# plume-sig/zk-nullifier-sig

Hardware: AMD Instinct MI355X
Metric: PLUME verifies/sec (secp256k1 V1) at batch=2^20 per GPU (higher is better)
Workload: dtype u32; 1 GPU; BASELINE.json configs[1]/metric: batch 2^20 per GPU, PLUME V1 verify (secp256k1 + SHA-256), 32-byte messages, 1/16 corrupted, inputs resident in HBM; Fp arithmetic on 9x29-bit limbs through chains of v_mad_u64_u32 (32x32+64); items_per_gpu=1048576, parallelism=shard x1, no collective on the data path, world_size=1

## Files before the change

__graft_entry__.py:

```python
import os
import subprocess
import sys
from pathlib import Path

ROOT = Path(__file__).resolve().parent
os.environ.setdefault("HSA_ENABLE_IPC_MODE_LEGACY", "0")
os.environ.setdefault("GPU_MAX_HW_QUEUES", "8")
if str(ROOT) not in sys.path:
    sys.path.insert(0, str(ROOT))


def build() -> None:
    env = dict(os.environ, PYTORCH_ROCM_ARCH="gfx950")
    subprocess.check_call(["make", "-j2", "-C", str(ROOT / "zk-nullifier-sig_amd" / "csrc")], env=env)
    subprocess.check_call(["make", "-C", str(ROOT / "oracle")])
    subprocess.check_call(["make", "-C", str(ROOT / "tests" / "devsim")])
    subprocess.check_call(["make", "-C", str(ROOT / "tests" / "devgpu")])
    import zk_nullifier_sig_amd as plume
    assert plume.library_path().exists()


def smoke() -> None:
    import numpy as np

    import zk_nullifier_sig_amd as plume
    from oracle import plume_oracle as O
    from tests import _oracle_c as OC
    from tests import synth

    eng = plume.Engine(0)
    n = 64
    for ver in (1, 2):
        b = synth.sign_inputs(n)
        got = eng.sign_batch(ver, b["msgs"], b["off"], b["sk"], b["r"])
        want = OC.sign_batch(ver, b["msgs"], b["off"], b["sk"], b["r"], nthreads=4)
        for k in got:
            assert np.array_equal(got[k], want[k]), f"sign v{ver}: {k} differs from the oracle"
        v = synth.corrupt_for_verify(ver, b, got)
        ok = eng.verify_batch(ver, v["msgs"], v["off"], v["pk"], v["nullifier"], v["c"], v["s"], v.get("r_point"), v.get("hashed_to_curve_r"))
        want_ok = OC.verify_batch(ver, v["msgs"], v["off"], v["pk"], v["nullifier"], v["c"], v["s"], v.get("r_point"), v.get("hashed_to_curve_r"), nthreads=4)
        assert np.array_equal(ok, want_ok), f"verify v{ver} differs from the oracle"
        assert list(ok) == [0 if i % 16 == 5 else 1 for i in range(n)]
        nz = (ver, b["msgs"], b["off"], got["pk"], got["nullifier"], got["s"], got["r_point"], got["hashed_to_curve_r"], got["c"])
        assert np.array_equal(eng.verify_non_zk_batch(*nz), OC.verify_non_zk_batch(*nz, nthreads=4)), f"verify_non_zk v{ver} differs from the oracle"

    class Mock:
        def fill_bytes(self, k):
            return bytes.fromhex("93b9323b629f251b8f3fc2dd11f4672c5544e8230d493eceea98a90bda789808")

    sk = plume.SecretKey.from_bytes(bytes.fromhex("519b423d715f8b581f4fa8ee59f4771a5b44c8130b4e3eacca54a56dda72b464"))
    sig = plume.PlumeSignature.sign_v1(sk, b"An example app message string", Mock(), eng)
    assert sig.c.to_bytes().hex() == "c6a7fc2c926ddbaf20731a479fb6566f2daa5514baae5223fe3b32edbce83254"
    assert sig.s.to_bytes().hex() == "e69f027d84cb6fe5f761e333d12e975fb190d163e8ea132d7de0bd6079ba28ca"
    assert sig.verify(eng)
    assert O.verify(1, sig.message, (sig.pk.x, sig.pk.y), (sig.nullifier.x, sig.nullifier.y), sig.c.value, sig.s.value,
                    (sig.v1specific.r_point.x, sig.v1specific.r_point.y), (sig.v1specific.hashed_to_curve_r.x, sig.v1specific.hashed_to_curve_r.y))
    eng.close()
    print("smoke ok:", plume.library_path())


if __name__ == "__main__":
    build() if (len(sys.argv) < 2 or sys.argv[1] == "build") else smoke()
```

zk-nullifier-sig_amd/csrc/plume_capi.hip:

```cpp
#include <hip/hip_runtime.h>

#include <sched.h>

#include <cctype>
#include <condition_variable>
#include <cstdio>
#include <cstdlib>
#include <cstring>
#include <functional>
#include <iterator>
#include <map>
#include <mutex>
#include <cerrno>
#include <sys/random.h>
#include <string>
#include <thread>
#include <tuple>
#include <initializer_list>
#include <algorithm>
#include <atomic>
#include <memory>
#include <vector>

#include "../../include/plume_hip.h"
// ... 672 lines not shown
}

struct RecoverCall {
    RecoverLaunch fn;
    int version, format;
    uint8_t *rpt, *hr, *h, *status;
};

static int verify_device(plume_ctx* ctx, int version, int mode, size_t n, const uint8_t* msgs, const uint64_t* msg_off, size_t msgs_bytes, const uint8_t* pk, const uint8_t* nul,
                         const uint8_t* c, const uint8_t* s, const uint8_t* rpt, const uint8_t* hr, uint8_t* ok, hipStream_t st,
                         const uint8_t* preflags = nullptr, bool continue_timer = false, const uint8_t* rpt33 = nullptr, const uint8_t* hr33 = nullptr,
                         const RecoverCall* rec = nullptr) {
    if (n == 0) return 0;
    if (n > ctx->chunk) return fail(PLUME_ERR_ARG, "n exceeds the chunk size (plume_set_chunk)");
    if (int rc = need_gtab(ctx)) return rc;
    const bool eq1short = verify_eq1_short(ctx, version, mode, n, rpt != nullptr && rpt33 == nullptr);
    if (eq1short) { if (int rc = need_gcomb(ctx)) return rc; }
    const size_t J = eq1short ? 4 : 3;
    if (!continue_timer) { if (int rc = ws_acquire(ctx, st)) return rc; }
    std::unique_ptr<WsHold> hold(continue_timer ? nullptr : new WsHold(ctx, st));
    const std::vector<size_t> cut = sub_batch_bounds(ctx, n);
    const size_t nsub = cut.size() - 1;
    const bool overlapped = nsub > 1;
    if (int rc = verify_workspace(ctx, n, J, cut)) return rc;
    if (overlapped) { if (int rc = pre_events(ctx, nsub)) return rc; if (int rc = pre_stream(ctx)) return rc; }
    StageTimer& t = ctx->timer;
    if (!continue_timer) t.begin(st);
    hipStream_t pre = overlapped ? ctx->pre : st;
    if (overlapped) {
        HIPCHK(hipEventRecord(ctx->pre_begin, st));
        HIPCHK(hipStreamWaitEvent(pre, ctx->pre_begin, 0));
    }
    for (size_t k = 0; k < nsub; k++) {
        const size_t lo = cut[k], cnt = cut[k + 1] - cut[k];
        VerifyArgs a;
        memset(&a, 0, sizeof a);
        a.version = version; a.mode = mode; a.n = (uint32_t)cnt; a.msgs = msgs; a.msg_off = msg_off + lo; a.msgs_bytes = msgs_bytes;
        a.pk = pk + 64 * lo; a.nul = nul + 64 * lo; a.c = c + 32 * lo; a.s = s + 32 * lo; a.rpt = rpt ? rpt + 64 * lo : nullptr; a.hr = hr ? hr + 64 * lo : nullptr; a.ok = ok ? ok + lo : nullptr;
        a.preflags = preflags ? preflags + lo : nullptr; a.rpt33 = rpt33 ? rpt33 + 33 * lo : nullptr; a.hr33 = hr33 ? hr33 + 33 * lo : nullptr;
        a.bases = ctx->bases.as<uint32_t>() + (size_t)PLUME_BASE_WORDS * J * lo; a.jobflags = ctx->jobflags.as<uint8_t>() + J * lo; a.itemflags = ctx->itemflags.as<uint8_t>() + lo;
        a.tab = ctx->tab.as<uint32_t>() + (size_t)PLUME_TAB_WORDS * J * lo; a.res = ctx->res.as<uint32_t>() + (size_t)PLUME_JAC_WORDS * 2 * lo; a.resinf = ctx->resinf.as<uint8_t>() + 2 * lo;
        a.gtab = ctx->fixed->gtab.as<uint32_t>();
        a.redo = ctx->redo.as<uint32_t>() + 2 * lo + k;
        a.digs = ctx->digs.as<int8_t>() + (size_t)PLUME_VDIG_ROWS * lo;
        if (eq1short) {
            a.eq1fall = ctx->eq1fall.as<uint8_t>() + lo; a.eq1k = ctx->eq1k.as<uint32_t>() + 8 * lo; a.gcomb = ctx->fixed->gcomb.as<uint32_t>();
            a.eq1force = ctx->eq1_short == 2 ? 1 : 0;
        }
        if (k == 0) ctx->redo_counters.clear();
        ctx->redo_counters.push_back(2 * lo + k);
        const bool two_roles = cnt <= ctx->ingest_split_max;
        a.msm_pair = (!eq1short && cnt <= ctx->msm_pair_max) ? 1 : 0;
        a.scalars_in_ingest = two_roles && ctx->split_scalars ? 1 : 0;
        launch_verify_ingest(a, pre, two_roles); if (!overlapped) t.stage(a.scalars_in_ingest ? "verify_ingest_h2c+scalars" : "verify_ingest_h2c", st);
        if (!a.scalars_in_ingest) { launch_verify_scalars(a, pre); if (!overlapped) t.stage("verify_scalars", st); }
        table_stage(ctx, a.tab, a.bases, a.jobflags, J * cnt, 3 * cnt, pre); if (!overlapped) t.stage("tables", st);
        if (overlapped) {
            HIPCHK(hipEventRecord(ctx->pre_ready[k], pre));
            HIPCHK(hipStreamWaitEvent(st, ctx->pre_ready[k], 0));
        }
        ctx->last_msm_kernel = verify_msm_kernel_name(a);
        if (k == 0) ctx->last_msm_sampled = false;
        if (t.on && !overlapped && k == 0) {
            if (ctx->clk.ensure(16)) return PLUME_ERR_HIP;
            HIPCHK(hipMemsetAsync(ctx->clk.p, 0, 16, st));
            a.clk = ctx->clk.as<unsigned long long>();
            ctx->last_msm_sampled = true;
        }
        launch_verify_msm(a, st); if (!overlapped) t.stage("verify_msm", st);
        if (version == 2 && mode == PLUME_MODE_VERIFY) { launch_normalize(a.res, a.resinf, 2 * cnt, st); if (!overlapped) t.stage("to_affine", st); }
        if (rec) {
            const size_t P = recover_width(rec->format);
            RecoverArgs ra;
            memset(&ra, 0, sizeof ra);
            ra.version = rec->version; ra.format = rec->format; ra.n = a.n; ra.pk = a.pk; ra.nul = a.nul; ra.c = a.c;
            ra.itemflags = a.itemflags; ra.jobflags = a.jobflags; ra.tab = a.tab; ra.res = a.res; ra.resinf = a.resinf;
            ra.rpt = rec->rpt ? rec->rpt + P * lo : nullptr; ra.hr = rec->hr ? rec->hr + P * lo : nullptr; ra.h = rec->h ? rec->h + P * lo : nullptr;
            ra.status = rec->status ? rec->status + lo : nullptr;
            rec->fn(ra, st); if (!overlapped) t.stage("recover_finalize", st);
        } else {
            launch_verify_finalize(a, st); if (!overlapped) t.stage("verify_finalize", st);
        }
    }
    if (overlapped) t.stage("verify_overlapped", st);
    HIPCHK(hipGetLastError());
    return hold ? hold->release() : 0;
}

static int sign_device(plume_ctx* ctx, int version, size_t n, const uint8_t* msgs, const uint64_t* msg_off, size_t msgs_bytes, const uint8_t* sk, const uint8_t* r,
                       const uint8_t* pk_in, uint8_t* pk, uint8_t* nul, uint8_t* c, uint8_t* s, uint8_t* rpt, uint8_t* hr, uint8_t* status, uint8_t* h_out,
                       hipStream_t st, bool out33 = false, const uint8_t* aux = nullptr, SignNonceLaunch nonce_fn = nullptr) {
    if (n == 0) return 0;
    if (n > ctx->chunk) return fail(PLUME_ERR_ARG, "n exceeds the chunk size (plume_set_chunk)");
    if (int rc = need_sign_tables(ctx)) return rc;
    const bool selfcheck = ctx->sign_selfcheck != 0;
    const SignReleaseLaunch release_fn = selfcheck ? g_sign_release.load() : nullptr;
    if (selfcheck && !release_fn) return fail(PLUME_ERR_ARG, "the signer's self-check is on but its release kernel is not part of this build");
    const bool sc_eq1short = selfcheck && verify_eq1_short(ctx, version, PLUME_MODE_NON_ZK, n, true);
    if (selfcheck) { if (int rc = need_fixed(ctx, true, sc_eq1short, false)) return rc; }
    if (int rc = ws_acquire(ctx, st)) return rc;
    WsHold hold(ctx, st);
    const std::vector<size_t> cut = sub_batch_bounds(ctx, n);
    constexpr size_t kStageBytes = 4 * 64 + 2 * 32 + 2;
    if (selfcheck && (verify_workspace(ctx, n, sc_eq1short ? 4 : 3, cut) || ctx->scstage.ensure(kStageBytes * n) || (ctx->timer.on && ctx->clk.ensure(16)))) return PLUME_ERR_HIP;
    uint8_t* const stg = ctx->scstage.as<uint8_t>();
    uint8_t *const g_pk = stg, *const g_nul = stg + 64 * n, *const g_rpt = stg + 128 * n, *const g_hr = stg + 192 * n, *const g_c = stg + 256 * n, *const g_s = stg + 288 * n,
            *const g_status = stg + 320 * n, *const g_ok = stg + 321 * n;
    struct StageWipe {
        plume_ctx* ctx; size_t bytes; hipStream_t st;
        ~StageWipe() { if (bytes) (void)hipMemsetAsync(ctx->scstage.p, 0, bytes, st); }
    } stage_wipe{ctx, selfcheck ? kStageBytes * n : 0, st};
    uint8_t *const u_pk = pk, *const u_nul = nul, *const u_c = c, *const u_s = s, *const u_rpt = rpt, *const u_hr = hr, *const u_status = status;
    const bool u_out33 = out33;
    if (selfcheck) { pk = g_pk; nul = g_nul; c = g_c; s = g_s; rpt = g_rpt; hr = g_hr; status = g_status; out33 = false; }
    const size_t nsub = cut.size() - 1;
    const bool overlapped = nsub > 1;
    size_t scr_bytes = 0;
    constexpr size_t SK = PLUME_SIGN_K;
    for (size_t k = 0; k < nsub; k++) scr_bytes = std::max(scr_bytes, table_stage_scratch(ctx, SK * (cut[k + 1] - cut[k]), 0));
    if (ctx->bases.ensure((size_t)PLUME_BASE_WORDS * 4 * SK * n) || ctx->jobflags.ensure(SK * n) || ctx->itemflags.ensure(n) || ctx->tab.ensure((size_t)PLUME_TAB_WORDS * 4 * SK * n) ||
// ... 1621 lines not shown
```

zk-nullifier-sig_amd/csrc/plume_ec.h:

```cpp
#pragma once
#include "plume_field.h"

#if !defined(__HIP_DEVICE_COMPILE__) && defined(PLUME_FE_CHECK)
namespace plume { inline unsigned long& fallback_counter() { static unsigned long c = 0; return c; } }
#define PLUME_COUNT_FALLBACK() (++plume::fallback_counter())
#else
#define PLUME_COUNT_FALLBACK() ((void)0)
#endif

namespace plume {

struct jac {
    fe x, y, z;
    uint32_t inf;
};

PLUME_HD fe fe_beta() { return fe_set(0x7AE96A2Bu, 0x657C0710u, 0x6E64479Eu, 0xAC3434E9u, 0x9CF04975u, 0x12F58995u, 0xC1396C28u, 0x719501EEu); }
PLUME_HD fe fe_gx() { return fe_set(0x79BE667Eu, 0xF9DCBBACu, 0x55A06295u, 0xCE870B07u, 0x029BFCDBu, 0x2DCE28D9u, 0x59F2815Bu, 0x16F81798u); }
PLUME_HD fe fe_gy() { return fe_set(0x483ADA77u, 0x26A3C465u, 0x5DA4FBFCu, 0x0E1108A8u, 0xFD17B448u, 0xA6855419u, 0x9C47D08Fu, 0xFB10D4B8u); }

PLUME_HD fe fe_off_x() { return fe_set(0xBE71E685u, 0x6986BD54u, 0xA5797708u, 0x9EF9F753u, 0x1397E48Bu, 0x08AA9EB1u, 0x128983CAu, 0x1D5B099Bu); }
PLUME_HD fe fe_off_y() { return fe_set(0x15AE5773u, 0x1FAF9233u, 0xF016B8C3u, 0x84D627FDu, 0x8CF7C500u, 0x22EAB6A1u, 0x27C3954Bu, 0x8A01ED04u); }
PLUME_HD fe fe_off_c128_x() { return fe_set(0x8141C548u, 0xF0861E56u, 0xAE562CECu, 0x00E54F8Bu, 0x7535C0B1u, 0x943A12D3u, 0x469080E1u, 0xA23EEBF9u); }
PLUME_HD fe fe_off_c128_y() { return fe_set(0xE429892Au, 0x9AB04F55u, 0xF3E86FE7u, 0xE225348Fu, 0xEF934040u, 0xDC585E87u, 0x1A3CC5BEu, 0x78194203u); }
// ... 173 lines not shown
#define PLUME_NDIG ((128 + PLUME_WBITS) / PLUME_WBITS)
#ifndef PLUME_GW
#define PLUME_GW 24
#endif
static_assert(PLUME_GW % PLUME_WBITS == 0, "a wide digit must line up with the windows of the shared doubling chain");
static_assert(PLUME_GW <= 24, "the digit rows hold a wide digit as a magnitude of up to three bytes plus its sign");
static_assert(PLUME_GW >= 16, "wide digits are stored as magnitude bytes + a sign byte: needs W / 4 >= 4 positions per digit");
#define PLUME_GW_BYTES (PLUME_GW > 16 ? 3 : 2)
#define PLUME_GWS (PLUME_GW / PLUME_WBITS)
#define PLUME_NDIGW ((128 + PLUME_GW) / PLUME_GW)
#define PLUME_GTAB_ENTRIES (1 << (PLUME_GW - 1))
PLUME_HD int booth_digit_w(const uint32_t m[4], int k) {
    const int W = PLUME_GW, lo = W * k - 1;
    const uint32_t mask = (1u << (W + 1)) - 1u;
    uint32_t u;
    if (lo < 0) {
        u = (m[0] << 1) & mask;
    } else {
        int wi = lo >> 5, sh = lo & 31;
        uint32_t a = wi < 4 ? m[wi] : 0u, b = (wi + 1) < 4 ? m[wi + 1] : 0u;
        u = ((a >> sh) | ((sh > 31 - W) ? (b << (32 - sh)) : 0u)) & mask;
    }
    return (int)(u & 1) + (int)((u >> 1) & ((1u << (W - 1)) - 1u)) - (int)((u >> W) << (W - 1));
}
PLUME_HD void booth_store_wide(int8_t* dig, uint32_t stride, const glv_half& h, bool flip) {
    bool neg = (h.neg != 0) != flip;
    PLUME_UNROLL for (int k = 0; k < PLUME_NDIGW; k++) {
        int d = booth_digit_w(h.m, k);
        bool dn = (d < 0) != neg;
        int mag = d < 0 ? -d : d;
        const int pos = PLUME_GWS * k;
        const int8_t sgn = (int8_t)((mag != 0 && dn) ? 1 : 0);
        static_assert(PLUME_GWS >= PLUME_GW_BYTES + 1, "a wide digit's bytes fit its positions");
        if (pos + PLUME_GW_BYTES < PLUME_NDIG) {
            PLUME_UNROLL for (int b = 0; b < PLUME_GW_BYTES; b++) dig[(uint32_t)(pos + b) * stride] = (int8_t)(uint8_t)((mag >> (8 * b)) & 0xFF);
            dig[(uint32_t)(pos + PLUME_GW_BYTES) * stride] = sgn;
        } else if (pos + 1 < PLUME_NDIG) {
            dig[(uint32_t)pos * stride] = (int8_t)(uint8_t)(mag & 0xFF);
            dig[(uint32_t)(pos + 1) * stride] = (int8_t)(uint8_t)(((mag >> 8) & 0x7F) | (sgn ? 0x80 : 0));
        } else {
            dig[(uint32_t)pos * stride] = (int8_t)(uint8_t)((mag & 0x3F) | (sgn ? 0x40 : 0));
        }
    }
}
#define PLUME_NPOS 65
#define PLUME_NPOS64 33
#define PLUME_NPOS66 34
#ifndef PLUME_SIGN_K
#define PLUME_SIGN_K 2
#endif
#define PLUME_SIGN_BITS (128 / PLUME_SIGN_K)
#define PLUME_NPOSK (PLUME_SIGN_BITS / 2 + 1)
static_assert(PLUME_SIGN_K == 2 || PLUME_SIGN_K == 4, "pieces of 64 or 32 bits (whole words of the GLV halves)");
PLUME_HD uint32_t eisd_entry_table(int ta, int tb) {
    static const uint16_t T[64] = {0x240, 0x343, 0x44F, 0x144, 0x261, 0x366, 0x469, 0x167, 0x28D, 0x38C, 0x492, 0x10B, 0x222, 0x328, 0x02A, 0x125,
                                   0x240, 0x343, 0x44F, 0x144, 0x261, 0x366, 0x469, 0x167, 0x28D, 0x38C, 0x011, 0x10B, 0x222, 0x328, 0x02A, 0x125,
                                   0x240, 0x343, 0x44F, 0x144, 0x261, 0x366, 0x469, 0x167, 0x28D, 0x38C, 0x011, 0x10B, 0x222, 0x328, 0x02A, 0x125,
                                   0x240, 0x343, 0x44F, 0x144, 0x261, 0x366, 0x469, 0x167, 0x28D, 0x38C, 0x011, 0x10B, 0x222, 0x328, 0x02A, 0x125};
    const uint32_t idx = (((uint32_t)ta & 3u) << 2) | ((uint32_t)tb & 3u) | (ta < 0 ? 16u : 0u) | (tb < 0 ? 32u : 0u);
    return T[idx];
}
PLUME_HD uint32_t eisd_entry(int ta, int tb) {
    const uint32_t i = (((uint32_t)ta & 3u) << 2) | ((uint32_t)tb & 3u);
    const uint64_t CLO = 0x5C98D3A4C123C60ull, CHI = 0x2A902ull, D0 = 0x2491246DB492ull, D1 = 0x21A31A31A31Aull;
    uint32_t code = (uint32_t)((i < 12u ? CLO >> (5u * i) : CHI >> (5u * (i - 12u))) & 31u);
    uint32_t d0 = (uint32_t)(D0 >> (3u * i)) & 7u, d1 = (uint32_t)(D1 >> (3u * i)) & 7u;
    if (i == 10u && (ta < 0 || tb < 0)) { code = 17u; d0 = 0u; d1 = 0u; }
    return code | (d0 << 5) | (d1 << 8);
}
template <int NP, int NW>
PLUME_HD bool eisd_store(int8_t* dig, uint32_t stride, const uint32_t (&am)[NW], bool aneg, const uint32_t (&bm)[NW], bool bneg, bool flip) {
    const int sa = (aneg != flip) ? -1 : 1, sb = (bneg != flip) ? -1 : 1;
    int ca = 0, cb = 0;
    PLUME_UNROLL for (int i = 0; i < NP; i++) {
        const int w = (2 * i) >> 5, sh = (2 * i) & 31;
        const int cha = w < NW ? (int)((am[w < NW ? w : 0] >> sh) & 3u) : 0, chb = w < NW ? (int)((bm[w < NW ? w : 0] >> sh) & 3u) : 0;
        const int ta = sa * cha + ca, tb = sb * chb + cb;
        const uint32_t e = eisd_entry(ta, tb);
        dig[(uint32_t)i * stride] = (int8_t)(e & 31u);
        ca = (ta - ((int)((e >> 5) & 7u) - 2)) >> 2;
        cb = (tb - ((int)((e >> 8) & 7u) - 2)) >> 2;
    }
    return ca == 0 && cb == 0;
}
PLUME_HD void eisd_store_glv(int8_t* dig, uint32_t stride, const glv_half& h1, const glv_half& h2, bool flip) {
    (void)eisd_store<PLUME_NPOS, 4>(dig, stride, h1.m, h1.neg != 0, h2.m, h2.neg != 0, flip);
}

#define PLUME_TAB_ENTRIES 3
#define PLUME_FE_W PLUME_FE_WORDS
#define PLUME_JAC_WORDS (3 * PLUME_FE_WORDS)
#define PLUME_TAB_ENTRY_WORDS 32
#define PLUME_TAB_WORDS (PLUME_TAB_ENTRIES * PLUME_TAB_ENTRY_WORDS)

PLUME_HD void ld_tab_xy(fe& x, fe& y, const uint32_t* e, bool lambda_half) {
    const uint32_t* xs = lambda_half ? e + 16 : e;
    PLUME_UNROLL for (int i = 0; i < 8; i++) { x.v[i] = xs[i]; y.v[i] = e[8 + i]; }
    x.v[8] = lambda_half ? e[26] : e[24];
    y.v[8] = e[25];
}
template <int ROWS>
PLUME_HD void ld_tab_xy_scan(fe& x, fe& y, const uint32_t* tab, int ad, bool lambda_half) {
    ld_tab_xy(x, y, tab, lambda_half);
    PLUME_NOUNROLL for (int e = 1; e < ROWS; e++) {
        fe rx, ry;
        ld_tab_xy(rx, ry, tab + (size_t)e * PLUME_TAB_ENTRY_WORDS, lambda_half);
        const bool take = ad == e + 1;
        fe_cmov(x, rx, take); fe_cmov(y, ry, take);
    }
}
PLUME_HD void st_tab_entry(uint32_t* e, const fe& x, const fe& y, const fe& bx) {
    PLUME_UNROLL for (int i = 0; i < 8; i++) { e[i] = x.v[i]; e[8 + i] = y.v[i]; e[16 + i] = bx.v[i]; }
    e[24] = x.v[8]; e[25] = y.v[8]; e[26] = bx.v[8]; e[27] = 0;
    e[28] = 0; e[29] = 0; e[30] = 0; e[31] = 0;
}
PLUME_HD void ld_fe(fe& r, const uint32_t* p) { PLUME_UNROLL for (int i = 0; i < PLUME_FE_W; i++) r.v[i] = p[i]; }
PLUME_HD void st_fe(uint32_t* p, const fe& a) { PLUME_UNROLL for (int i = 0; i < PLUME_FE_W; i++) p[i] = a.v[i]; }
PLUME_HD void ld_fe_soa(fe& r, const uint32_t* base, size_t stride, size_t j) { PLUME_UNROLL for (int i = 0; i < PLUME_FE_W; i++) r.v[i] = base[(size_t)i * stride + j]; }
PLUME_HD void st_fe_soa(uint32_t* base, size_t stride, size_t j, const fe& a) { PLUME_UNROLL for (int i = 0; i < PLUME_FE_W; i++) base[(size_t)i * stride + j] = a.v[i]; }
PLUME_HD void ld_jac_soa(jac& p, const uint32_t* base, size_t stride, size_t j) {
    ld_fe_soa(p.x, base, stride, j); ld_fe_soa(p.y, base + PLUME_FE_W * stride, stride, j); ld_fe_soa(p.z, base + 2 * PLUME_FE_W * stride, stride, j);
}
PLUME_HD void st_jac_soa(uint32_t* base, size_t stride, size_t j, const jac& p) {
    st_fe_soa(base, stride, j, p.x); st_fe_soa(base + PLUME_FE_W * stride, stride, j, p.y); st_fe_soa(base + 2 * PLUME_FE_W * stride, stride, j, p.z);
}
#define PLUME_BASE_WORDS 28
struct alignas(16) quad32 { uint32_t a, b, c, d; };
PLUME_HD void st_base(uint32_t* bases, size_t job, const jac& p) {
    quad32* q = reinterpret_cast<quad32*>(bases + job * PLUME_BASE_WORDS);
    q[0] = quad32{p.x.v[0], p.x.v[1], p.x.v[2], p.x.v[3]}; q[1] = quad32{p.x.v[4], p.x.v[5], p.x.v[6], p.x.v[7]};
    q[2] = quad32{p.x.v[8], p.y.v[0], p.y.v[1], p.y.v[2]}; q[3] = quad32{p.y.v[3], p.y.v[4], p.y.v[5], p.y.v[6]};
    q[4] = quad32{p.y.v[7], p.y.v[8], p.z.v[0], p.z.v[1]}; q[5] = quad32{p.z.v[2], p.z.v[3], p.z.v[4], p.z.v[5]};
    q[6] = quad32{p.z.v[6], p.z.v[7], p.z.v[8], 0u};
}
PLUME_HD void ld_base(jac& p, const uint32_t* bases, size_t job, bool with_z) {
    const quad32* q = reinterpret_cast<const quad32*>(bases + job * PLUME_BASE_WORDS);
    const quad32 q0 = q[0], q1 = q[1], q2 = q[2], q3 = q[3], q4 = q[4];
    p.x.v[0] = q0.a; p.x.v[1] = q0.b; p.x.v[2] = q0.c; p.x.v[3] = q0.d; p.x.v[4] = q1.a; p.x.v[5] = q1.b; p.x.v[6] = q1.c; p.x.v[7] = q1.d; p.x.v[8] = q2.a;
    p.y.v[0] = q2.b; p.y.v[1] = q2.c; p.y.v[2] = q2.d; p.y.v[3] = q3.a; p.y.v[4] = q3.b; p.y.v[5] = q3.c; p.y.v[6] = q3.d; p.y.v[7] = q4.a; p.y.v[8] = q4.b;
    if (with_z) {
// ... 457 lines not shown
```

zk-nullifier-sig_amd/csrc/plume_kernels.hip:

```cpp
#include <algorithm>

#include "plume_launch.h"
#include "plume_dedup.h"

#define PLUME_MIN_WAVES 4
#define PLUME_MSM_WAVES PLUME_MIN_WAVES
#define PLUME_H2C_WAVES 3
#define PLUME_FINAL_WAVES 2
#define PLUME_NORM_WAVES 2
#define PLUME_BOUNDS __launch_bounds__(kBlock, PLUME_MIN_WAVES)
#define PLUME_FINAL_BOUNDS __launch_bounds__(kBlock, PLUME_FINAL_WAVES)
#define PLUME_NORM_BOUNDS __launch_bounds__(kBlock, PLUME_NORM_WAVES)
#define PLUME_MSM_BOUNDS __launch_bounds__(kBlock, PLUME_MSM_WAVES)
#define PLUME_H2C_BOUNDS __launch_bounds__(kBlock, PLUME_H2C_WAVES)

namespace plume {



__global__ PLUME_BOUNDS void k_fixed_bases(uint32_t* base18, uint32_t nwin, uint32_t W) {
    const uint32_t w = blockIdx.x * kBlock + threadIdx.x;
    if (w < nwin) fixed_window_base(base18 + (size_t)w * 2 * PLUME_FE_W, W * w);
}
__global__ PLUME_BOUNDS void k_fixed_table(uint32_t* rows, const uint32_t* base18, uint32_t entries, uint32_t nwin) {
    const size_t lane = (size_t)blockIdx.x * kBlock + threadIdx.x;
    if (lane < (size_t)entries * nwin) fixed_table_lane(rows, base18, entries, lane);
}

__global__ __launch_bounds__(kBlock, 4) void k_verify_scalars(VerifyArgs a) {
    const uint32_t i = blockIdx.x * kBlock + threadIdx.x;
    if (i == 0) a.redo[0] = 0;
    if (i < a.n) verify_scalars(a, i);
}

__global__ PLUME_H2C_BOUNDS void k_verify_ingest(VerifyArgs a) {
    uint32_t i = blockIdx.x * kBlock + threadIdx.x;
    if (i < a.n) verify_ingest_h2c(a, i);
}

__global__ PLUME_H2C_BOUNDS void k_verify_ingest_split(VerifyArgs a) {
    constexpr uint32_t H = kBlock / 2;
    __shared__ uint32_t s_u1[PLUME_FE_WORDS * H];
    __shared__ uint32_t s_q[3 * PLUME_FE_WORDS * H];
    __shared__ uint32_t s_fb[H];
    const uint32_t l = threadIdx.x & (H - 1);
    const bool roleB = threadIdx.x >= H;
    const uint32_t i = blockIdx.x * H + l;
    const bool live = i < a.n;
    if (a.scalars_in_ingest && blockIdx.x == 0 && threadIdx.x == H) a.redo[0] = 0;
    ingest_xch x;
    ingest_a_state st;
    if (live) {
        if (roleB) { verify_ingest_b1(a, i, x); s_fb[l] = x.fb; }
        else { verify_ingest_a1(a, i, x, st); PLUME_UNROLL for (int k = 0; k < PLUME_FE_WORDS; k++) s_u1[k * H + l] = x.u1.v[k]; }
    }
    __syncthreads();
    if (live) {
        if (roleB) {
            PLUME_UNROLL for (int k = 0; k < PLUME_FE_WORDS; k++) x.u1.v[k] = s_u1[k * H + l];
            verify_ingest_b2(x);
            PLUME_UNROLL for (int k = 0; k < PLUME_FE_WORDS; k++) { s_q[k * H + l] = x.xn.v[k]; s_q[(PLUME_FE_WORDS + k) * H + l] = x.xd.v[k]; s_q[(2 * PLUME_FE_WORDS + k) * H + l] = x.y.v[k]; }
        } else {
            x.fb = s_fb[l];
            verify_ingest_a2(a, i, x, st);
        }
    }
    __syncthreads();
    if (live && !roleB) {
        PLUME_UNROLL for (int k = 0; k < PLUME_FE_WORDS; k++) { x.xn.v[k] = s_q[k * H + l]; x.xd.v[k] = s_q[(PLUME_FE_WORDS + k) * H + l]; x.y.v[k] = s_q[(2 * PLUME_FE_WORDS + k) * H + l]; }
        verify_ingest_a3(a, i, x, st);
    } else if (live && a.scalars_in_ingest) {
        verify_scalars(a, i);
    }
}

struct WaveRowSink {
    uint4* rows;
    uint32_t** ptrs;
    bool full;
    __device__ void sync() const { __builtin_amdgcn_fence(__ATOMIC_ACQ_REL, "wavefront"); __builtin_amdgcn_wave_barrier(); }
    __device__ void operator()(uint32_t* e, const fe& x, const fe& y, const fe& bx) const {
        if (!full) { st_tab_entry(e, x, y, bx); return; }
        const uint32_t lane = threadIdx.x & 63u, sw = lane & 7u;
        uint4* mine = rows + lane * 8;
        mine[0 ^ sw] = make_uint4(x.v[0], x.v[1], x.v[2], x.v[3]);
        mine[1 ^ sw] = make_uint4(x.v[4], x.v[5], x.v[6], x.v[7]);
        mine[2 ^ sw] = make_uint4(y.v[0], y.v[1], y.v[2], y.v[3]);
        mine[3 ^ sw] = make_uint4(y.v[4], y.v[5], y.v[6], y.v[7]);
        mine[4 ^ sw] = make_uint4(bx.v[0], bx.v[1], bx.v[2], bx.v[3]);
        mine[5 ^ sw] = make_uint4(bx.v[4], bx.v[5], bx.v[6], bx.v[7]);
        mine[6 ^ sw] = make_uint4(x.v[8], y.v[8], bx.v[8], 0u);
        mine[7 ^ sw] = make_uint4(0u, 0u, 0u, 0u);
        ptrs[lane] = e;
        __builtin_amdgcn_fence(__ATOMIC_RELEASE, "wavefront");
        __builtin_amdgcn_wave_barrier();
        __builtin_amdgcn_fence(__ATOMIC_ACQUIRE, "wavefront");
        const uint32_t quad = lane & 7u;
        PLUME_UNROLL for (uint32_t q = 0; q < 8; q++) {
            const uint32_t r = (lane >> 3) + 8u * q;
            const uint4 v = rows[r * 8 + (quad ^ (r & 7u))];
            reinterpret_cast<uint4*>(ptrs[r])[quad] = v;
        }
        __builtin_amdgcn_fence(__ATOMIC_RELEASE, "wavefront");
        __builtin_amdgcn_wave_barrier();
    }
};

#define PLUME_TABPASS_WAVES_A 4
#define PLUME_TABPASS_WAVES_B 3
#define PLUME_TABINV_K 8
constexpr int kTabBlock = 128;
__global__ __launch_bounds__(kTabBlock, PLUME_TABPASS_WAVES_A) void k_tab_pass_a(const uint32_t* bases, const uint8_t* jobflags, size_t njobs, int L, uint32_t* scr, uint32_t* carry, uint8_t* guardf) {
    const size_t lane = (size_t)blockIdx.x * kTabBlock + threadIdx.x, nl = (size_t)gridDim.x * kTabBlock;
    const size_t j0 = lane * (size_t)L;
    const int cnt = j0 < njobs ? (int)((njobs - j0) < (size_t)L ? (njobs - j0) : (size_t)L) : 0;
    uint32_t* myscr = scr + (size_t)blockIdx.x * ((size_t)L * PLUME_TAB_SCR_WORDS * kTabBlock);
    fe c;
    bool g = false;
    tab_pass_a(bases, jobflags, njobs, j0, cnt, myscr, (size_t)kTabBlock, threadIdx.x, c, g);
    st_fe_soa(carry, nl, lane, c); guardf[lane] = g ? 1 : 0;
}
__global__ __launch_bounds__(kTabBlock, PLUME_TABPASS_WAVES_B) void k_tab_pass_b(uint32_t* tab, const uint32_t* bases, const uint8_t* jobflags, size_t njobs, int L, const uint32_t* scr, const uint32_t* carry,
                                                                                  const uint8_t* guardf) {
    __shared__ uint4 s_rows[kTabBlock * 8];
    __shared__ uint32_t* s_ptrs[kTabBlock];
// ... 370 lines not shown
```

zk-nullifier-sig_amd/csrc/plume_stages.h:

```cpp
#pragma once
#include "plume_h2c.h"
#include "plume_eis.h"

namespace plume {

PLUME_HD uint32_t load_affine_be(fe& x, fe& y, const uint8_t* p) {
    uint32_t wx[8], wy[8];
    words_from_be_aligned(wx, p);
    words_from_be_aligned(wy, p + 32);
    fe_from_words(x, wx);
    fe_from_words(y, wy);
    uint32_t nz = 0;
    PLUME_UNROLL for (int i = 0; i < 8; i++) nz |= wx[i] | wy[i];
    if (nz == 0) return PLUME_JOB_INF;
    if (!words_lt_p(wx) || !words_lt_p(wy)) return PLUME_JOB_INVALID;
    return affine_on_curve(x, y) ? PLUME_JOB_OK : PLUME_JOB_INVALID;
}
PLUME_HD uint32_t reload_affine_be(fe& x, fe& y, const uint8_t* p) {
    uint32_t wx[8], wy[8];
    words_from_be_aligned(wx, p);
    words_from_be_aligned(wy, p + 32);
    fe_from_words(x, wx);
    fe_from_words(y, wy);
    uint32_t nz = 0;
// ... 75 lines not shown
    const bool ok = o1 >= o0 && o1 <= msgs_bytes && o1 - o0 <= 0xFFFFFF00ull;
    len = ok ? (uint32_t)(o1 - o0) : 0u;
    if (!ok) o0 = 0;
    return ok;
}

#define PLUME_MODE_VERIFY 0
#define PLUME_MODE_NON_ZK 1
#define PLUME_ITEM_REJECT 1u
#define PLUME_ITEM_ERR 2u
struct VerifyArgs {
    int version;
    int mode;
    uint32_t n;
    const uint8_t* msgs; const uint64_t* msg_off;
    uint64_t msgs_bytes;
    const uint8_t *pk, *nul, *c, *s, *rpt, *hr;
    uint8_t* ok;
    const uint8_t* preflags;
    const uint8_t *rpt33, *hr33;
    uint32_t* bases;
    uint8_t* jobflags;
    uint8_t* itemflags;
    uint32_t* tab;
    uint32_t* res;
    uint8_t* resinf;
    const uint32_t* gtab;
    uint32_t* redo;
    int8_t* digs;
    uint8_t* eq1fall;
    uint32_t* eq1k;
    const uint32_t* gcomb;
    int msm_pair;
    int scalars_in_ingest;
    unsigned long long* clk;
    int eq1force;
};
PLUME_HD bool verify_eq1_short(const VerifyArgs& a) { return a.eq1fall != nullptr; }
PLUME_HD size_t verify_njobs(const VerifyArgs& a) { return (verify_eq1_short(a) ? 4 : 3) * (size_t)a.n; }
#define PLUME_VDIG_SET PLUME_NPOS
#define PLUME_VDIG_SETB (2 * PLUME_NPOS66)
#define PLUME_VDIG_ROWS (2 * PLUME_VDIG_SET + PLUME_VDIG_SETB)
static_assert(PLUME_VDIG_SETB >= 2 * PLUME_NDIG, "set B holds either form");
PLUME_HD uint32_t redo_file(uint32_t* redo, uint32_t task) {
#if defined(__HIP_DEVICE_COMPILE__)
    const uint32_t k = atomicAdd(redo, 1u);
#else
    const uint32_t k = redo[0]++;
#endif
    redo[1 + k] = task;
    return k;
}

PLUME_HD void verify_item_digits(int8_t* d, uint32_t n, const sc& s, const glv_half& c1, const glv_half& c2, bool long_b) {
    glv_half h1, h2;
    glv_split(h1, h2, s);
    eisd_store_glv(d, n, h1, h2, false);
    if (long_b) { booth_store_wide(d + (size_t)PLUME_VDIG_SET * n, n, h1, false); booth_store_wide(d + (size_t)(PLUME_VDIG_SET + PLUME_NDIG) * n, n, h2, false); }
    eisd_store_glv(d + (size_t)(PLUME_VDIG_SET + PLUME_VDIG_SETB) * n, n, c1, c2, true);
}
PLUME_HD void verify_scalars(const VerifyArgs& a, uint32_t i) {
    sc c, s;
    bool okc = load_scalar_be(c, a.c + 32 * (size_t)i), oks = load_scalar_be(s, a.s + 32 * (size_t)i);
    if (a.mode == PLUME_MODE_NON_ZK) { okc = sc_lt_n(c); oks = sc_lt_n(s); }
    if (!okc || !oks) { if (verify_eq1_short(a)) a.eq1fall[i] = 1; return; }
    bool lng = true;
    glv_half c1, c2;
    glv_split(c1, c2, c);
    if (verify_eq1_short(a)) {
        eis_short e;
        eis_half_gcd(e, c1, c2);
        lng = !e.ok || a.eq1force != 0 || !eis_consistent(e, c);
        if (!lng) {
            sc k;
            sc_mul(k, e.tau, s);
            PLUME_UNROLL for (int w = 0; w < 8; w++) a.eq1k[(size_t)w * a.n + i] = k.v[w];
            int8_t* b = a.digs + (size_t)PLUME_VDIG_SET * a.n + i;
            (void)eisd_store<PLUME_NPOS66, 3>(b, a.n, e.u[0], e.uneg[0] != 0, e.u[1], e.uneg[1] != 0, true);
            (void)eisd_store<PLUME_NPOS66, 3>(b + (size_t)PLUME_NPOS66 * a.n, a.n, e.t[0], e.tneg[0] != 0, e.t[1], e.tneg[1] != 0, true);
        }
        a.eq1fall[i] = lng ? 1 : 0;
    }
    verify_item_digits(a.digs + i, a.n, s, c1, c2, lng);
}

PLUME_HD void verify_ingest_h2c(const VerifyArgs& a, uint32_t i) {
    fe pkx, pky, nx, ny;
    uint32_t fpk = load_affine_be(pkx, pky, a.pk + 64 * (size_t)i);
    uint32_t fnul = load_affine_be(nx, ny, a.nul + 64 * (size_t)i);
    sc c, s;
    bool okc = load_scalar_be(c, a.c + 32 * (size_t)i), oks = load_scalar_be(s, a.s + 32 * (size_t)i);
    if (a.mode == PLUME_MODE_NON_ZK) { okc = sc_lt_n(c); oks = sc_lt_n(s); }
    uint64_t o0; uint32_t mlen;
    const bool okm = msg_span(o0, mlen, a.msg_off, i, a.msgs_bytes);
    bool bad = !okc || !oks || !okm || fpk == PLUME_JOB_INVALID || fnul == PLUME_JOB_INVALID || (a.preflags && a.preflags[i]);
    const bool err = a.mode == PLUME_MODE_NON_ZK && !bad && fpk == PLUME_JOB_INF;
    a.itemflags[i] = (uint8_t)(bad ? PLUME_ITEM_REJECT : err ? PLUME_ITEM_ERR : 0u);
    bad = bad || err;
    if (verify_eq1_short(a)) {
        fe rx, ry;
        const uint32_t fr = load_affine_be(rx, ry, a.rpt + 64 * (size_t)i);
        if (fr == PLUME_JOB_INVALID && !err) { bad = true; a.itemflags[i] = (uint8_t)PLUME_ITEM_REJECT; }
        jac p; p.inf = 0; p.z = fe_small(1); p.x = rx; p.y = ry;
        st_base(a.bases, 3 * (size_t)a.n + i, p); a.jobflags[3 * (size_t)a.n + i] = (uint8_t)(fr | PLUME_JOB_AFFINE);
    }
    {
        jac p; p.inf = 0; p.z = fe_small(1);
        p.x = nx; p.y = ny;
        st_base(a.bases, 3 * (size_t)i + 2, p); a.jobflags[3 * (size_t)i + 2] = (uint8_t)(fnul | PLUME_JOB_AFFINE);
        p.x = pkx; p.y = pky;
        st_base(a.bases, 3 * (size_t)i + 0, p); a.jobflags[3 * (size_t)i + 0] = (uint8_t)(fpk | PLUME_JOB_AFFINE);
    }
    const uint32_t pktag = 2u + (fe_is_odd(pky) ? 1u : 0u);
    jac h;
    if (!bad) {
        hash_to_curve_jac(h, a.msgs + o0, mlen, pkx, pktag, fpk == PLUME_JOB_INF ? PLUME_ENC_IDENTITY : PLUME_ENC_POINT);
    } else {
        h.x = fe_gx(); h.y = fe_gy(); h.z = fe_small(1); h.inf = 0;
    }
    st_base(a.bases, 3 * (size_t)i + 1, h); a.jobflags[3 * (size_t)i + 1] = (uint8_t)(h.inf ? PLUME_JOB_INF : PLUME_JOB_OK);
}

struct ingest_xch {
    fe u1;
    uint32_t fb;
    fe xn, xd, y;
};
struct ingest_a_state { fe u0; fe c, d, y1; uint32_t fpk; bool bad_a, bad; };
PLUME_HD void verify_ingest_b1(const VerifyArgs& a, uint32_t i, ingest_xch& x) {
    fe nx, ny;
    const uint32_t fnul = load_affine_be(nx, ny, a.nul + 64 * (size_t)i);
    sc c, s;
    bool okc = load_scalar_be(c, a.c + 32 * (size_t)i), oks = load_scalar_be(s, a.s + 32 * (size_t)i);
    if (a.mode == PLUME_MODE_NON_ZK) { okc = sc_lt_n(c); oks = sc_lt_n(s); }
    jac p; p.inf = 0; p.z = fe_small(1); p.x = nx; p.y = ny;
    st_base(a.bases, 3 * (size_t)i + 2, p); a.jobflags[3 * (size_t)i + 2] = (uint8_t)(fnul | PLUME_JOB_AFFINE);
// ... 560 lines not shown
```

Baseline: 56.72 million verifies/s.

## Recode scalar digits with an LDS-resident carry state machine table

Replaces the per-digit joint recoding of GLV/Eisenstein scalar halves with a precomputed finite-state-machine table that folds the carry into the state. The table is built at compile time, copied into shared memory per block, and several digit chains are interleaved so independent lookups can overlap. The clock reset moves from a host memset into the scalar kernel. This trades ALU work in the scalar stage for LDS lookups and a block-wide table copy plus a barrier. The scalar stage is likely a small share of total verify time next to the MSM.

```diff
diff --git a/__graft_entry__.py b/__graft_entry__.py
--- a/__graft_entry__.py
+++ b/__graft_entry__.py
@@ -16,6 +16,8 @@
     subprocess.check_call(["make", "-C", str(ROOT / "oracle")])
     subprocess.check_call(["make", "-C", str(ROOT / "tests" / "devsim")])
     subprocess.check_call(["make", "-C", str(ROOT / "tests" / "devgpu")])
+    subprocess.check_call(["make", "-C", str(ROOT / "tests" / "scalar_stage")])
+    subprocess.check_call(["make", "-C", str(ROOT / "tests" / "devgpu_recode")])
     import zk_nullifier_sig_amd as plume
     assert plume.library_path().exists()
 
diff --git a/zk-nullifier-sig_amd/csrc/plume_capi.hip b/zk-nullifier-sig_amd/csrc/plume_capi.hip
--- a/zk-nullifier-sig_amd/csrc/plume_capi.hip
+++ b/zk-nullifier-sig_amd/csrc/plume_capi.hip
@@ -748,20 +748,19 @@
         const bool two_roles = cnt <= ctx->ingest_split_max;
         a.msm_pair = (!eq1short && cnt <= ctx->msm_pair_max) ? 1 : 0;
         a.scalars_in_ingest = two_roles && ctx->split_scalars ? 1 : 0;
+        ctx->last_msm_kernel = verify_msm_kernel_name(a);
+        if (k == 0) ctx->last_msm_sampled = false;
+        if (t.on && !overlapped && k == 0) {
+            if (ctx->clk.ensure(16)) return PLUME_ERR_HIP;
+            a.clk = ctx->clk.as<unsigned long long>();
+            ctx->last_msm_sampled = true;
+        }
         launch_verify_ingest(a, pre, two_roles); if (!overlapped) t.stage(a.scalars_in_ingest ? "verify_ingest_h2c+scalars" : "verify_ingest_h2c", st);
         if (!a.scalars_in_ingest) { launch_verify_scalars(a, pre); if (!overlapped) t.stage("verify_scalars", st); }
         table_stage(ctx, a.tab, a.bases, a.jobflags, J * cnt, 3 * cnt, pre); if (!overlapped) t.stage("tables", st);
         if (overlapped) {
             HIPCHK(hipEventRecord(ctx->pre_ready[k], pre));
             HIPCHK(hipStreamWaitEvent(st, ctx->pre_ready[k], 0));
-        }
-        ctx->last_msm_kernel = verify_msm_kernel_name(a);
-        if (k == 0) ctx->last_msm_sampled = false;
-        if (t.on && !overlapped && k == 0) {
-            if (ctx->clk.ensure(16)) return PLUME_ERR_HIP;
-            HIPCHK(hipMemsetAsync(ctx->clk.p, 0, 16, st));
-            a.clk = ctx->clk.as<unsigned long long>();
-            ctx->last_msm_sampled = true;
         }
         launch_verify_msm(a, st); if (!overlapped) t.stage("verify_msm", st);
         if (version == 2 && mode == PLUME_MODE_VERIFY) { launch_normalize(a.res, a.resinf, 2 * cnt, st); if (!overlapped) t.stage("to_affine", st); }
diff --git a/zk-nullifier-sig_amd/csrc/plume_ec.h b/zk-nullifier-sig_amd/csrc/plume_ec.h
--- a/zk-nullifier-sig_amd/csrc/plume_ec.h
+++ b/zk-nullifier-sig_amd/csrc/plume_ec.h
@@ -249,13 +249,15 @@
 #define PLUME_SIGN_BITS (128 / PLUME_SIGN_K)
 #define PLUME_NPOSK (PLUME_SIGN_BITS / 2 + 1)
 static_assert(PLUME_SIGN_K == 2 || PLUME_SIGN_K == 4, "pieces of 64 or 32 bits (whole words of the GLV halves)");
-PLUME_HD uint32_t eisd_entry_table(int ta, int tb) {
-    static const uint16_t T[64] = {0x240, 0x343, 0x44F, 0x144, 0x261, 0x366, 0x469, 0x167, 0x28D, 0x38C, 0x492, 0x10B, 0x222, 0x328, 0x02A, 0x125,
-                                   0x240, 0x343, 0x44F, 0x144, 0x261, 0x366, 0x469, 0x167, 0x28D, 0x38C, 0x011, 0x10B, 0x222, 0x328, 0x02A, 0x125,
-                                   0x240, 0x343, 0x44F, 0x144, 0x261, 0x366, 0x469, 0x167, 0x28D, 0x38C, 0x011, 0x10B, 0x222, 0x328, 0x02A, 0x125,
-                                   0x240, 0x343, 0x44F, 0x144, 0x261, 0x366, 0x469, 0x167, 0x28D, 0x38C, 0x011, 0x10B, 0x222, 0x328, 0x02A, 0x125};
+namespace eisd_detail {
+constexpr static const uint16_t T[64] = {0x240, 0x343, 0x44F, 0x144, 0x261, 0x366, 0x469, 0x167, 0x28D, 0x38C, 0x492, 0x10B, 0x222, 0x328, 0x02A, 0x125,
+                                         0x240, 0x343, 0x44F, 0x144, 0x261, 0x366, 0x469, 0x167, 0x28D, 0x38C, 0x011, 0x10B, 0x222, 0x328, 0x02A, 0x125,
+                                         0x240, 0x343, 0x44F, 0x144, 0x261, 0x366, 0x469, 0x167, 0x28D, 0x38C, 0x011, 0x10B, 0x222, 0x328, 0x02A, 0x125,
+                                         0x240, 0x343, 0x44F, 0x144, 0x261, 0x366, 0x469, 0x167, 0x28D, 0x38C, 0x011, 0x10B, 0x222, 0x328, 0x02A, 0x125};
+}
+PLUME_HD constexpr uint32_t eisd_entry_table(int ta, int tb) {
     const uint32_t idx = (((uint32_t)ta & 3u) << 2) | ((uint32_t)tb & 3u) | (ta < 0 ? 16u : 0u) | (tb < 0 ? 32u : 0u);
-    return T[idx];
+    return eisd_detail::T[idx];
 }
 PLUME_HD uint32_t eisd_entry(int ta, int tb) {
     const uint32_t i = (((uint32_t)ta & 3u) << 2) | ((uint32_t)tb & 3u);
@@ -283,6 +285,79 @@
 PLUME_HD void eisd_store_glv(int8_t* dig, uint32_t stride, const glv_half& h1, const glv_half& h2, bool flip) {
     (void)eisd_store<PLUME_NPOS, 4>(dig, stride, h1.m, h1.neg != 0, h2.m, h2.neg != 0, flip);
 }
+constexpr int kEisdFsmStates = 9, kEisdFsmQuadrant = kEisdFsmStates * 16, kEisdFsmEntries = 4 * kEisdFsmQuadrant;
+constexpr uint32_t kEisdFsmRest = 4u << 5;
+struct eisd_fsm { uint16_t e[kEisdFsmEntries]; };
+constexpr eisd_fsm eisd_fsm_build() {
+    eisd_fsm t{};
+    for (int q = 0; q < 4; q++) for (int st = 0; st < kEisdFsmStates; st++) for (int ch = 0; ch < 16; ch++) {
+        const int sa = (q & 1) ? -1 : 1, sb = (q & 2) ? -1 : 1, ca = st / 3 - 1, cb = st % 3 - 1;
+        const int ta = sa * (ch >> 2) + ca, tb = sb * (ch & 3) + cb;
+        const uint32_t e = eisd_entry_table(ta, tb);
+        const int na = (ta - ((int)((e >> 5) & 7u) - 2)) >> 2, nb = (tb - ((int)((e >> 8) & 7u) - 2)) >> 2;
+        const int ns = (na < -1 || na > 1 || nb < -1 || nb > 1) ? 15 : 3 * (na + 1) + (nb + 1);
+        t.e[q * kEisdFsmQuadrant + st * 16 + ch] = (uint16_t)((e & 31u) | ((uint32_t)ns << 5));
+    }
+    return t;
+}
+constexpr bool eisd_fsm_closed(const eisd_fsm& t) {
+    for (int k = 0; k < kEisdFsmEntries; k++) if ((t.e[k] >> 5) >= kEisdFsmStates) return false;
+    return true;
+}
+static_assert(eisd_fsm_closed(eisd_fsm_build()), "the recoding's carries stay in {-1, 0, 1}");
+PLUME_HD const uint16_t* eisd_fsm_table() {
+    static constexpr eisd_fsm T = eisd_fsm_build();
+    return T.e;
+}
+template <int NW>
+struct eisd_fsm_chain {
+    uint32_t am[NW], bm[NW];
+    const uint16_t* tab;
+    uint32_t st;
+    int8_t* dig;
+};
+template <int NW>
+PLUME_HD void eisd_fsm_begin(eisd_fsm_chain<NW>& c, const uint16_t* tab, int8_t* dig, const uint32_t (&am)[NW], bool aneg, const uint32_t (&bm)[NW], bool bneg, bool flip) {
+    PLUME_UNROLL for (int w = 0; w < NW; w++) { c.am[w] = am[w]; c.bm[w] = bm[w]; }
+    c.tab = tab + ((aneg != flip) ? kEisdFsmQuadrant : 0) + ((bneg != flip) ? 2 * kEisdFsmQuadrant : 0);
+    c.st = kEisdFsmRest;
+    c.dig = dig;
+}
+template <int NW>
+PLUME_HD void eisd_fsm_step(eisd_fsm_chain<NW>& c, int i, uint32_t stride) {
+    const int w = (2 * i) >> 5, sh = (2 * i) & 31;
+    const uint32_t cha = w < NW ? (c.am[w < NW ? w : 0] >> sh) & 3u : 0u, chb = w < NW ? (c.bm[w < NW ? w : 0] >> sh) & 3u : 0u;
+    const uint32_t e = *reinterpret_cast<const uint16_t*>(reinterpret_cast<const char*>(c.tab) + (c.st + 2u * ((cha << 2) | chb)));
+    c.dig[(uint32_t)i * stride] = (int8_t)(e & 31u);
+    c.st = e & ~31u;
+}
+template <int NW>
+PLUME_HD bool eisd_fsm_done(const eisd_fsm_chain<NW>& c) { return c.st == kEisdFsmRest; }
+template <int NP, int NW>
+PLUME_HD bool eisd_store_fsm(const uint16_t* tab, int8_t* dig, uint32_t stride, const uint32_t (&am)[NW], bool aneg, const uint32_t (&bm)[NW], bool bneg, bool flip) {
+    eisd_fsm_chain<NW> c;
+    eisd_fsm_begin(c, tab, dig, am, aneg, bm, bneg, flip);
+    PLUME_UNROLL for (int i = 0; i < NP; i++) eisd_fsm_step(c, i, stride);
+    return eisd_fsm_done(c);
+}
+template <int NP, int NW>
+PLUME_HD void eisd_fsm_walk2(eisd_fsm_chain<NW>& x, eisd_fsm_chain<NW>& y, uint32_t stride) {
+    PLUME_UNROLL for (int i = 0; i < NP; i++) { eisd_fsm_step(x, i, stride); eisd_fsm_step(y, i, stride); }
+}
+template <int NPA, int NWA, int NPB, int NWB>
+PLUME_HD void eisd_fsm_walk4(eisd_fsm_chain<NWA>& x, eisd_fsm_chain<NWA>& y, eisd_fsm_chain<NWB>& u, eisd_fsm_chain<NWB>& v, uint32_t stride) {
+    static_assert(NPB <= NPA, "the short pairs end first");
+    PLUME_UNROLL for (int i = 0; i < NPA; i++) {
+        eisd_fsm_step(x, i, stride); eisd_fsm_step(y, i, stride);
+        if (i < NPB) { eisd_fsm_step(u, i, stride); eisd_fsm_step(v, i, stride); }
+    }
+}
+#if defined(__HIPCC__) || defined(__HIP__)
+__device__ __forceinline__ void eisd_fsm_to_lds(uint16_t* s_tab) {
+    const uint16_t* t = eisd_fsm_table();
+    for (uint32_t k = threadIdx.x; k < (uint32_t)kEisdFsmEntries; k += blockDim.x) s_tab[k] = t[k];
+}
+#endif
 
 #define PLUME_TAB_ENTRIES 3
 #define PLUME_FE_W PLUME_FE_WORDS
diff --git a/zk-nullifier-sig_amd/csrc/plume_kernels.hip b/zk-nullifier-sig_amd/csrc/plume_kernels.hip
--- a/zk-nullifier-sig_amd/csrc/plume_kernels.hip
+++ b/zk-nullifier-sig_amd/csrc/plume_kernels.hip
@@ -27,10 +27,17 @@
     if (lane < (size_t)entries * nwin) fixed_table_lane(rows, base18, entries, lane);
 }
 
+__device__ __forceinline__ void verify_scalars_once(const VerifyArgs& a) {
+    a.redo[0] = 0;
+    if (a.clk != nullptr) { a.clk[0] = 0; a.clk[1] = 0; }
+}
 __global__ __launch_bounds__(kBlock, 4) void k_verify_scalars(VerifyArgs a) {
+    __shared__ uint16_t s_fsm[kEisdFsmEntries];
     const uint32_t i = blockIdx.x * kBlock + threadIdx.x;
-    if (i == 0) a.redo[0] = 0;
-    if (i < a.n) verify_scalars(a, i);
+    if (i == 0) verify_scalars_once(a);
+    eisd_fsm_to_lds(s_fsm);
+    __syncthreads();
+    if (i < a.n) verify_scalars(a, i, s_fsm);
 }
 
 __global__ PLUME_H2C_BOUNDS void k_verify_ingest(VerifyArgs a) {
@@ -43,11 +50,13 @@
     __shared__ uint32_t s_u1[PLUME_FE_WORDS * H];
     __shared__ uint32_t s_q[3 * PLUME_FE_WORDS * H];
     __shared__ uint32_t s_fb[H];
+    __shared__ uint16_t s_fsm[kEisdFsmEntries];
     const uint32_t l = threadIdx.x & (H - 1);
     const bool roleB = threadIdx.x >= H;
     const uint32_t i = blockIdx.x * H + l;
     const bool live = i < a.n;
-    if (a.scalars_in_ingest && blockIdx.x == 0 && threadIdx.x == H) a.redo[0] = 0;
+    if (a.scalars_in_ingest && blockIdx.x == 0 && threadIdx.x == H) verify_scalars_once(a);
+    if (a.scalars_in_ingest) eisd_fsm_to_lds(s_fsm);
     ingest_xch x;
     ingest_a_state st;
     if (live) {
@@ -70,7 +79,7 @@
         PLUME_UNROLL for (int k = 0; k < PLUME_FE_WORDS; k++) { x.xn.v[k] = s_q[k * H + l]; x.xd.v[k] = s_q[(PLUME_FE_WORDS + k) * H + l]; x.y.v[k] = s_q[(2 * PLUME_FE_WORDS + k) * H + l]; }
         verify_ingest_a3(a, i, x, st);
     } else if (live && a.scalars_in_ingest) {
-        verify_scalars(a, i);
+        verify_scalars(a, i, s_fsm);
     }
 }
 
diff --git a/zk-nullifier-sig_amd/csrc/plume_stages.h b/zk-nullifier-sig_amd/csrc/plume_stages.h
--- a/zk-nullifier-sig_amd/csrc/plume_stages.h
+++ b/zk-nullifier-sig_amd/csrc/plume_stages.h
@@ -151,36 +151,47 @@
     return k;
 }
 
-PLUME_HD void verify_item_digits(int8_t* d, uint32_t n, const sc& s, const glv_half& c1, const glv_half& c2, bool long_b) {
+PLUME_HD void verify_item_digits(int8_t* d, uint32_t n, const sc& s, const glv_half& c1, const glv_half& c2, bool long_b, const uint16_t* fsm = eisd_fsm_table()) {
     glv_half h1, h2;
     glv_split(h1, h2, s);
-    eisd_store_glv(d, n, h1, h2, false);
+    eisd_fsm_chain<4> ds, dc;
+    eisd_fsm_begin(ds, fsm, d, h1.m, h1.neg != 0, h2.m, h2.neg != 0, false);
+    eisd_fsm_begin(dc, fsm, d + (size_t)(PLUME_VDIG_SET + PLUME_VDIG_SETB) * n, c1.m, c1.neg != 0, c2.m, c2.neg != 0, true);
     if (long_b) { booth_store_wide(d + (size_t)PLUME_VDIG_SET * n, n, h1, false); booth_store_wide(d + (size_t)(PLUME_VDIG_SET + PLUME_NDIG) * n, n, h2, false); }
-    eisd_store_glv(d + (size_t)(PLUME_VDIG_SET + PLUME_VDIG_SETB) * n, n, c1, c2, true);
-}
-PLUME_HD void verify_scalars(const VerifyArgs& a, uint32_t i) {
+    eisd_fsm_walk2<PLUME_NPOS>(ds, dc, n);
+}
+PLUME_HD void verify_scalars(const VerifyArgs& a, uint32_t i, const uint16_t* fsm = eisd_fsm_table()) {
     sc c, s;
     bool okc = load_scalar_be(c, a.c + 32 * (size_t)i), oks = load_scalar_be(s, a.s + 32 * (size_t)i);
     if (a.mode == PLUME_MODE_NON_ZK) { okc = sc_lt_n(c); oks = sc_lt_n(s); }
     if (!okc || !oks) { if (verify_eq1_short(a)) a.eq1fall[i] = 1; return; }
-    bool lng = true;
     glv_half c1, c2;
     glv_split(c1, c2, c);
+    const uint32_t n = a.n;
+    int8_t* d = a.digs + i;
     if (verify_eq1_short(a)) {
         eis_short e;
         eis_half_gcd(e, c1, c2);
-        lng = !e.ok || a.eq1force != 0 || !eis_consistent(e, c);
+        const bool lng = !e.ok || a.eq1force != 0 || !eis_consistent(e, c);
+        a.eq1fall[i] = lng ? 1 : 0;
         if (!lng) {
             sc k;
             sc_mul(k, e.tau, s);
-            PLUME_UNROLL for (int w = 0; w < 8; w++) a.eq1k[(size_t)w * a.n + i] = k.v[w];
-            int8_t* b = a.digs + (size_t)PLUME_VDIG_SET * a.n + i;
-            (void)eisd_store<PLUME_NPOS66, 3>(b, a.n, e.u[0], e.uneg[0] != 0, e.u[1], e.uneg[1] != 0, true);
-            (void)eisd_store<PLUME_NPOS66, 3>(b + (size_t)PLUME_NPOS66 * a.n, a.n, e.t[0], e.tneg[0] != 0, e.t[1], e.tneg[1] != 0, true);
+            PLUME_UNROLL for (int w = 0; w < 8; w++) a.eq1k[(size_t)w * n + i] = k.v[w];
+            glv_half h1, h2;
+            glv_split(h1, h2, s);
+            int8_t* b = d + (size_t)PLUME_VDIG_SET * n;
+            eisd_fsm_chain<4> ds, dc;
+            eisd_fsm_chain<3> du, dt;
+            eisd_fsm_begin(ds, fsm, d, h1.m, h1.neg != 0, h2.m, h2.neg != 0, false);
+            eisd_fsm_begin(dc, fsm, d + (size_t)(PLUME_VDIG_SET + PLUME_VDIG_SETB) * n, c1.m, c1.neg != 0, c2.m, c2.neg != 0, true);
+            eisd_fsm_begin(du, fsm, b, e.u[0], e.uneg[0] != 0, e.u[1], e.uneg[1] != 0, true);
+            eisd_fsm_begin(dt, fsm, b + (size_t)PLUME_NPOS66 * n, e.t[0], e.tneg[0] != 0, e.t[1], e.tneg[1] != 0, true);
+            eisd_fsm_walk4<PLUME_NPOS, 4, PLUME_NPOS66, 3>(ds, dc, du, dt, n);
+            return;
         }
-        a.eq1fall[i] = lng ? 1 : 0;
-    }
-    verify_item_digits(a.digs + i, a.n, s, c1, c2, lng);
+    }
+    verify_item_digits(d, n, s, c1, c2, true, fsm);
 }
 
 PLUME_HD void verify_ingest_h2c(const VerifyArgs& a, uint32_t i) {
```

New measurement: 56.51 million verifies/s, median of 2. Within noise of the previous version (-0.4%).
